# huggingface/distil-whisper

Hardware: AMD Instinct MI355X
Metric: training audio-seconds/s (distil-large-v3 student, 30 s clips) (higher is better)
Workload: dtype bf16

## Files before the change

### distil_whisper_amd/build.py

```python
import os
import subprocess
import sys

HERE = os.path.dirname(os.path.abspath(__file__))
CSRC = os.path.join(HERE, "csrc")
LIB = os.path.join(HERE, "libdwamd.so")
SOURCES = ["gemm.hip", "gemm_tile256.hip", "gemm_tile128.hip", "gemm_wp8_nn.hip", "gemm_wp8_nt.hip", "gemm_wp8_m320.hip", "gemm_wp8_m128.hip",
           "gemm_wp16_nn.hip", "gemm_wp16_tt.hip", "gemm_wp16_small.hip", "gemm_skinny.hip", "attention.hip", "norm.hip", "loss.hip", "logmel.hip", "elementwise.hip", "optim.hip", "decode.hip", "align.hip", "score.hip", "dropout.hip"]
FLAGS = ["--offload-arch=gfx950", "-O3", "-std=c++17", "-fPIC", "-ffp-contract=fast", "-munsafe-fp-atomics"]


def kernels_sha16() -> str:
    import hashlib
    h = hashlib.sha256()
    files = sorted(os.path.join(CSRC, f) for f in os.listdir(CSRC) if f.endswith((".hip", ".h")))
    files.append(os.path.join(HERE, "..", "include", "dwamd.h"))
    for f in files:
        h.update(os.path.basename(f).encode())
        with open(f, "rb") as fh:
            h.update(fh.read())
    return h.hexdigest()[:16]


def _stale(obj, deps):
    if not os.path.exists(obj):
        return True
    t = os.path.getmtime(obj)
    return any(os.path.getmtime(d) > t for d in deps)


# ... 33 lines not shown
```

### distil_whisper_amd/csrc/gemm.hip

```cpp
#include "gemm_common.h"
#include <mutex>
#include <unordered_map>

bool dw_gemm_skinny_ok(const GemmP& p, int trans_a, int trans_b);
int dw_gemm_skinny_launch(const GemmP& p, hipStream_t s);
int dw_gemm_tile256_launch(const GemmP& p, int ta, int tb, hipStream_t s);
int dw_gemm_tile128_launch(const GemmP& p, int ta, int tb, hipStream_t s);
int dw_gemm_wp8_nn_launch(const GemmP& p, hipStream_t s);
int dw_gemm_wp8_nt_launch(const GemmP& p, hipStream_t s);
int dw_gemm_wp8_nn320_launch(const GemmP& p, hipStream_t s);
int dw_gemm_wp8_nt320_launch(const GemmP& p, hipStream_t s);
int dw_gemm_wp8_nn128_launch(const GemmP& p, hipStream_t s);
int dw_gemm_wp8_nt128_launch(const GemmP& p, hipStream_t s);
int dw_gemm_wp16_nn_launch(const GemmP& p, hipStream_t s);
int dw_gemm_wp16_tt_launch(const GemmP& p, hipStream_t s);
int dw_gemm_wp16_nn_small_launch(const GemmP& p, hipStream_t s);
int dw_gemm_wp16_nt_small_launch(const GemmP& p, hipStream_t s);

extern int g_attn_bwd_stage;
extern int g_attn_decode;
extern int g_attn_ablate;
extern int g_attn_fwd_waves;
extern int g_attn_fwd_pipe;
extern int g_attn_plain_order;
extern int g_attn_defer;
extern int g_attn_bwd_waves;
extern int g_logmel_mfma;
extern int g_decode_fuse_off;
extern int g_skinny_wide;
extern int g_ln_variant;
enum { GEMM_RULE = 0,
       GEMM_REFERENCE = 1,
       GEMM_FORCE_320 = 2 };
static int g_gemm_mode = GEMM_RULE;
int g_gemm_strip = 0;
int g_gemm_cus = 256;
static int g_gemm_stage_next = 1;
static int g_gemm_dynamic = 1;
static int g_gemm_small_m = 1;
static int g_gemm_row_tail = 1;

static int* gemm_sched_slot(hipStream_t s) {
    static std::mutex mu;
    static std::unordered_map<hipStream_t, int*> slots;
    std::lock_guard<std::mutex> lock(mu);
    auto it = slots.find(s);
    if (it != slots.end()) return it->second;
    hipStreamCaptureStatus st = hipStreamCaptureStatusNone;
    if (hipStreamIsCapturing(s, &st) != hipSuccess || st != hipStreamCaptureStatusNone) { (void)hipGetLastError(); return nullptr; }
    int* ptr = nullptr;
    if (hipMalloc((void**)&ptr, 64) != hipSuccess || hipMemsetAsync(ptr, 0, 64, s) != hipSuccess) { (void)hipGetLastError(); return nullptr; }
    slots[s] = ptr;
    return ptr;
}
int g_gemm_strip_budget = 4;
extern "C" int dw_debug_set(int key, int value) {
    if (key == 0) { if (value < GEMM_RULE || value > GEMM_FORCE_320) return DW_EINVAL; g_gemm_mode = value; return DW_OK; }
    if (key == 1) { g_gemm_strip = value; return DW_OK; }
    if (key == 3) { g_attn_bwd_stage = value; return DW_OK; }
    if (key == 4) { g_attn_decode = value; return DW_OK; }
    if (key == 5) { g_logmel_mfma = value; return DW_OK; }
    if (key == 6) { g_gemm_strip_budget = value; return DW_OK; }
    if (key == 7) { g_decode_fuse_off = value; return DW_OK; }
    if (key == 8) { g_skinny_wide = value; return DW_OK; }
    if (key == 10) { g_gemm_dynamic = value; return DW_OK; }
    if (key == 11) { g_gemm_stage_next = value; return DW_OK; }
    if (key == 17) { g_attn_bwd_waves = value; return DW_OK; }
    if (key == 21) { g_ln_variant = value; return DW_OK; }
    if (key == 22) { g_gemm_row_tail = value; return DW_OK; }
    if (key == 25) { if (value < 0 || value > 1) return DW_EINVAL; g_gemm_small_m = value; return DW_OK; }
    if (key == 26) { g_attn_fwd_pipe = value; return DW_OK; }
    if (key == 18) { g_attn_plain_order = value; return DW_OK; }
    if (key == 23) { if (value < 0 || value > 64) return DW_EINVAL; g_attn_defer = value; return DW_OK; }
    if (key == 16) { g_attn_fwd_waves = value; return DW_OK; }
    if (key == 15) { g_attn_ablate = value; return DW_OK; }
    if (key == 9) { if (value < 8 || value > 256 || (value & 7)) return DW_EINVAL; g_gemm_cus = value; return DW_OK; }
    return DW_EINVAL;
}

__global__ __launch_bounds__(256) void reduce_slices_kernel(const float* part, long stride, int slices, float* out,
                                                            long n, int accumulate) {
    const long i = ((long)blockIdx.x * 256 + threadIdx.x) * 4;
    if (i >= n) return;
    f32x4 acc = accumulate ? *(const f32x4*)(out + i) : f32x4{0.f, 0.f, 0.f, 0.f};
    for (int s = 0; s < slices; ++s) {
        const f32x4 v = *(const f32x4*)(part + s * stride + i);
#pragma unroll
        for (int e = 0; e < 4; ++e) acc[e] += v[e];
    }
    *(f32x4*)(out + i) = acc;
}

// ... 28 lines not shown
                                   int rows, int cols, int accumulate, void* stream) {
    DW_CLEAR_ERR();
    if (!part || !out || slices < 1 || rows <= 0 || cols <= 0 || (cols & 3) || (ld_part & 3) || (ld_out & 3) || (slice_stride & 3) ||
        ld_part < cols || ld_out < cols || ((uintptr_t)part & 15) || ((uintptr_t)out & 15))
        return DW_EINVAL;
    const long n = (long)rows * (cols / 4);
    hipLaunchKernelGGL(reduce_slices_ld_kernel, dim3((n + 255) / 256), dim3(256), 0, (hipStream_t)stream, part, (long)slice_stride,
                       (long)ld_part, slices, out, (long)ld_out, rows, cols / 4, accumulate);
    DW_CHECK_LAUNCH();
    return DW_OK;
}

enum GemmKernel {
    K_SKINNY,
    K_TILE128,
    K_TILE256,
    K_WP8_M128,
    K_WP16_SMALL,
    K_WP8_320,
    K_WP16_NN,
    K_WP8_NN,
    K_WP8_NT,
    K_WP16_TT,
};

static GemmKernel gemm_choose(const DwGemm* g, const GemmP& p) {
    const bool ta = g->trans_a, tb = g->trans_b, nn = !ta && !tb;
    const bool one_slice = p.split_k == 1 && !p.atomic;
    const bool ref = g_gemm_mode == GEMM_REFERENCE;
    const bool res_f32 = g->r && g->r_dtype == DW_F32 && g->c_dtype == DW_F32;
    const long cus = g_gemm_cus, tn = (g->n + 255) / 256;
    const long t256 = (long)((g->m + 255) / 256) * tn;
    const bool fits320 = !ta && one_slice && g->m % 320 == 0 && g->n % 256 == 0;
    int tile = g->tile;
    if ((tile == 0 || tile == 16) && dw_gemm_skinny_ok(p, ta, tb)) return K_SKINNY;
    bool one_round_320 = false, small_m_256 = false;
    if (tile != 128 && tile != 256) {
        tile = t256 >= 512 ? 256 : 128;
        if (tile == 128 && !ref && g_gemm_small_m && !ta && one_slice) {
            const long r128 = (((long)(g->m + 127) / 128) * tn + cus - 1) / cus;
            const long r256 = (t256 + cus - 1) / cus;
            const long r320 = fits320 ? ((long)(g->m / 320) * tn + cus - 1) / cus : 0;
            const long c128 = r128 * 100, c256 = r256 * 165, c320 = fits320 ? r320 * 205 : (1L << 40);
            if (c320 <= c128 && c320 <= c256) { tile = 256; one_round_320 = true; }
            else if (c256 <= c128) { tile = 256; small_m_256 = true; }
            else return K_WP8_M128;
        }
    }
    if (tile == 256 && g->tile != 256 && nn && res_f32 && g->k <= 1024 && one_slice) tile = 128;
    if (tile == 128) return K_TILE128;
    const long spanA = ta ? (long)g->k * g->lda * 2 : 256L * g->lda * 2 + (long)g->k * 2;
    const long spanB = tb ? (long)g->k * g->ldb * 2 : 256L * g->ldb * 2 + (long)g->k * 2;
    if (ref || spanA >= 0x7fffffffL || spanB >= 0x7fffffffL) return K_TILE256;
    if (small_m_256) return K_WP16_SMALL;
    if (fits320 && (one_round_320 || g_gemm_mode == GEMM_FORCE_320)) return K_WP8_320;
    if (nn && g->k <= 2560 && g->n >= 3840 && !g->r && !g->z_out && !g->zgrad_in && g->c_dtype != DW_F32) return K_WP16_NN;
    if (fits320) {
        const long r256 = (((g->m + 255) / 256) * tn + cus - 1) / cus * 4;
        const long r320 = ((g->m / 320) * tn + cus - 1) / cus * 5;
        if (tb ? r320 < r256 && !g->zgrad_in : r320 <= r256) return K_WP8_320;
    }
    if (nn) return res_f32 && g->k <= 2560 ? K_TILE256 : K_WP8_NN;
    if (!ta) return K_WP8_NT;
    if (tb) return K_WP16_TT;
    return K_TILE256;
}

extern "C" int dw_gemm_bf16(const DwGemm* g, void* stream) {
    DW_CLEAR_ERR();
    if (!g || (!g->a && !g->ln_x) || !g->b || !g->c) return DW_EINVAL;
    if (g->m <= 0 || g->n <= 0 || g->k <= 0 || (g->k & 63)) return DW_EINVAL;
    if ((g->lda & 7) || (g->ldb & 7)) return DW_EINVAL;
    if ((g->a && ((uintptr_t)g->a & 15)) || ((uintptr_t)g->b & 15)) return DW_EINVAL;
    if (g->trans_a && g->lda < ((g->m + 7) & ~7)) return DW_EINVAL;
    if (g->trans_b && g->ldb < ((g->n + 7) & ~7)) return DW_EINVAL;
    GemmP p;
    p.a = (const bf16*)g->a; p.b = (const bf16*)g->b; p.c = g->c; p.bias = g->bias;
    p.z_out = (bf16*)g->z_out; p.zgrad = (const bf16*)g->zgrad_in; p.r = g->r;
    p.lda = g->lda; p.ldb = g->ldb; p.ldc = g->ldc; p.ldz = g->ldz; p.ldzg = g->ldzg; p.ldr = g->ldr;
    p.m = g->m; p.n = g->n; p.k = g->k;
    p.act = g->act; p.c_dtype = g->c_dtype; p.r_dtype = g->r_dtype; p.r_row_mod = g->r_row_mod;
    p.round_res = g->round_res; p.tiles_n = 0; p.nwg = 0;
    p.split_k = g->split_k > 1 ? g->split_k : 1;
    p.atomic = g->atomic_acc ? 1 : 0;
    if (p.split_k > (g->k >> 6)) p.split_k = g->k >> 6;
    p.slice_stride = 0;
    p.sched = nullptr;
// ... 29 lines not shown
        if (g->r) v = v && ((uintptr_t)g->r % (g->r_dtype == DW_F32 ? 16 : 8)) == 0 && (g->ldr & 3) == 0;
        p.vec = v ? 1 : 0;
    }
    hipStream_t s = (hipStream_t)stream;
    if (g->tile == 16 && !dw_gemm_skinny_ok(p, g->trans_a, g->trans_b)) return DW_EINVAL;
    const GemmKernel kern = gemm_choose(g, p);
    if (kern == K_SKINNY) {
        if (g->colsum_out) return DW_EINVAL;
        return dw_gemm_skinny_launch(p, s);
    }
    if (fused) return DW_EINVAL;
    if (g->tile == 129 && (g->trans_a || p.split_k != 1 || p.atomic)) return DW_EINVAL;
    if (kern == K_TILE128) return dw_gemm_tile128_launch(p, g->trans_a, g->trans_b, s);
    p.strip = g_gemm_strip;
    if (g_gemm_dynamic) p.sched = gemm_sched_slot(s);
    if (kern == K_WP8_M128) return g->trans_b ? dw_gemm_wp8_nt128_launch(p, s) : dw_gemm_wp8_nn128_launch(p, s);
    if (g->k <= 1024) p.stage_next |= 128;
    switch (kern) {
    case K_WP16_SMALL: return g->trans_b ? dw_gemm_wp16_nt_small_launch(p, s) : dw_gemm_wp16_nn_small_launch(p, s);
    case K_WP8_320: return g->trans_b ? dw_gemm_wp8_nt320_launch(p, s) : dw_gemm_wp8_nn320_launch(p, s);
    case K_WP8_NN: return dw_gemm_wp8_nn_launch(p, s);
    case K_WP8_NT: return dw_gemm_wp8_nt_launch(p, s);
    case K_WP16_TT: return dw_gemm_wp16_tt_launch(p, s);
    case K_WP16_NN: {
        const int tm_full = p.m / 256, rem = p.m - tm_full * 256;
        const long tn = (p.n + 255) / 256;
        const long rounds_all = ((long)(tm_full + 1) * tn + g_gemm_cus - 1) / g_gemm_cus;
        const long rounds_full = ((long)tm_full * tn + g_gemm_cus - 1) / g_gemm_cus;
        if (g_gemm_row_tail && g->tile != 256 && rem > 0 && rem <= 128 && tm_full > 0 && rounds_full < rounds_all && !p.colsum) {
            GemmP q1 = p, q2 = p;
            q1.m = tm_full * 256;
            const size_t es = p.c_dtype == DW_F32 ? 4 : 2;
            q2.m = rem;
            q2.a = p.a + (long)q1.m * p.lda;
            q2.c = (char*)p.c + (size_t)q1.m * p.ldc * es;
            q2.sched = nullptr;
            const int rc1 = dw_gemm_wp16_nn_launch(q1, s);
            if (rc1 != DW_OK) return rc1;
            return dw_gemm_tile128_launch(q2, 0, 0, s);
        }
        return dw_gemm_wp16_nn_launch(p, s);
    }
    default: return dw_gemm_tile256_launch(p, g->trans_a, g->trans_b, s);
    }
}
```

### distil_whisper_amd/csrc/gemm_common.h

```cpp
#pragma once
#include "common.h"
#include "../../include/dwamd.h"

struct GemmP {
    const bf16* a;
    const bf16* b;
    void* c;
    const float* bias;
    bf16* z_out;
    const bf16* zgrad;
    const void* r;
    long lda, ldb, ldc, ldz, ldzg, ldr;
    int m, n, k;
    int act, c_dtype, r_dtype, r_row_mod, round_res;
    int tiles_n, nwg;
    int strip;
    int split_k, atomic;
    int vec;
    long slice_stride;
    const void* ln_x;
    const float* ln_g;
    const float* ln_b;
    long ld_lnx;
    int ln_x_dtype;
// ... 87 lines not shown
    int strip = id / per_strip;
    int within = id - strip * per_strip;
    int width = sw;
    const int full = p.tiles_n - (nstrips - 1) * sw;
    if (strip >= nstrips - 1) {
        strip = nstrips - 1;
        within = id - strip * per_strip;
        width = full;
    }
    tm = within / width;
    tn = strip * sw + (within - tm * width);
}

extern int g_gemm_strip_budget;
extern int g_gemm_cus;
inline int gemm_strip_width(int k, int tiles_n, int override_) {
    if (override_ > 0) return override_;
    const long tile_bytes = 256L * k * 2;
    int sw = (int)(((long)g_gemm_strip_budget << 19) / tile_bytes);
    if (sw < 2 || sw >= tiles_n) sw = tiles_n;
    return sw;
}

template <int BX>
__device__ __forceinline__ bf16x8 frag_kmajor(const char* tile, int x, int kk, int lane) {
    constexpr int RB = BX * 2;
    const int g = lane >> 4, p = lane & 15;
    const int col = x + ((g & 1) << 4) + ((p & 3) << 2);
    const int k0 = kk * 16 + ((g >> 1) << 3) + (p >> 2);
    const int ls = col >> 3;
    const int inb = (p & 1) << 3;
    const int sw = ((p >> 2) & 3) << 2;
    const char* a0 = tile + k0 * RB + ((ls ^ sw) << 4) + inb;
    const char* a1 = a0 + 4 * RB;
    bf16x4 lo = __builtin_amdgcn_ds_read_tr16_b64_v4bf16((lds_bf16x4_t*)a0);
    bf16x4 hi = __builtin_amdgcn_ds_read_tr16_b64_v4bf16((lds_bf16x4_t*)a1);
    bf16x8 r;
    r[0] = lo[0]; r[1] = lo[1]; r[2] = lo[2]; r[3] = lo[3];
    r[4] = hi[0]; r[5] = hi[1]; r[6] = hi[2]; r[7] = hi[3];
    return r;
}


typedef __attribute__((ext_vector_type(4))) unsigned u32x4;
enum { EPI_BIAS = 1, EPI_ZBF16 = 2, EPI_GELU = 4, EPI_STOREG = 8, EPI_ZG16 = 16, EPI_ZGBF = 32, EPI_RES = 64, EPI_RES_F32 = 128,
       EPI_ROUND = 256, EPI_OUT_F32 = 512, EPI_COLSUM = 1024 };
__device__ __forceinline__ int gemm_epi_flavour(const GemmP& p) {
    return (p.bias ? EPI_BIAS : 0) | ((p.z_out && !p.zg_f16) ? EPI_ZBF16 : 0) | (p.act == 1 ? EPI_GELU : 0) |
           ((p.z_out && p.zg_f16) ? EPI_STOREG : 0) | ((p.zgrad && p.zg_f16) ? EPI_ZG16 : 0) |
           ((p.zgrad && !p.zg_f16) ? EPI_ZGBF : 0) | (p.r ? EPI_RES : 0) | ((p.r && p.r_dtype == DW_F32) ? EPI_RES_F32 : 0) |
           ((p.r && p.round_res) ? EPI_ROUND : 0) | (p.c_dtype == DW_F32 ? EPI_OUT_F32 : 0) | (p.colsum ? EPI_COLSUM : 0);
}
template <class T>
__device__ __forceinline__ void gemm_store_out(T* dst, const T& v) {
    __builtin_nontemporal_store(v, dst);
// ... 82 lines not shown
    }
}

template <int LPR>
__device__ __forceinline__ void gemm_colsum_flush(const GemmP& p, float (&cs)[4], int lane, int n) {
#pragma unroll
    for (int e = 0; e < 4; ++e) {
#pragma unroll
        for (int o = LPR; o < 64; o <<= 1) cs[e] += __shfl_xor(cs[e], o);
    }
    if (lane < LPR) {
#pragma unroll
        for (int e = 0; e < 4; ++e)
            if (n + e < p.n) atomicAdd(p.colsum + n + e, cs[e]);
    }
}

struct GemmNoHook { __device__ __forceinline__ void operator()() const {} };
__device__ __forceinline__ void gemm_lds_barrier() {
    asm volatile("s_waitcnt lgkmcnt(0)" ::: "memory");
    __builtin_amdgcn_s_barrier();
    asm volatile("" ::: "memory");
}
template <int FM, int FN, int TN, int PFDIST = 0, class Hook = GemmNoHook, bool SWZ = false, int LAY = 32, int JOFF = 0, class Acc = f32x16[FM][FN]>
__device__ __forceinline__ void gemm_epilogue(const GemmP& p, Acc& acc, char* smem, int wave, int lane,
                                              int m0_, int wm0_, int n0_, int wn0_, int ks_, Hook hook = Hook(),
                                              const float* lds_bias = nullptr) {
    static_assert(!SWZ || TN == 64, "swizzled patch: 16 slots of 16 bytes per row");
    asm volatile("" : "+v"(lane));
    const int m0 = __builtin_amdgcn_readfirstlane(m0_), wm0 = __builtin_amdgcn_readfirstlane(wm0_);
    const int n0 = __builtin_amdgcn_readfirstlane(n0_), wn0 = __builtin_amdgcn_readfirstlane(wn0_);
    const int ks = __builtin_amdgcn_readfirstlane(ks_);
    constexpr int PLD = SWZ ? TN : TN + 4;
    constexpr int LPR = TN / 4;
    constexpr int RPI = 64 / LPR;
    constexpr int NIT = 32 / RPI;
    float* patch = (float*)smem + wave * (32 * PLD);
    const int hi = lane >> 5, ln = lane & 31;
    const int lrow = LAY == 32 ? ln : (lane & 15);
    const int lcol = LAY == 32 ? hi * 4 : (lane >> 4) * 4;
    auto qrow = [](int q) constexpr -> int { return LAY == 32 ? 0 : (q / (FN * 2)) * 16; };
    auto qcol = [](int q) constexpr -> int { return LAY == 32 ? (q / 4) * 32 + (q % 4) * 8 : (q % (FN * 2)) * 16; };
    auto quad = [&](auto ic, auto qc) __attribute__((always_inline)) -> f32x4 {
        constexpr int i = decltype(ic)::value, q = decltype(qc)::value;
        f32x4 v4;
        if constexpr (LAY == 32) {
            constexpr int j = q / 4, g = q % 4;
// ... 178 lines not shown
                    const bf16x2 r0 = __builtin_convertvector(p[0], bf16x2), r1 = __builtin_convertvector(p[1], bf16x2);
                    u32x2 o;
                    o[0] = __builtin_bit_cast(unsigned, r0); o[1] = __builtin_bit_cast(unsigned, r1);
                    *(u32x2*)(wr + qrow(q) * PRS + qcol(q) * 2) = o;
                });
                });
                flush(c_u, p.ldc, l_c16, ic);
                if constexpr (HAS_G) {
                    static_for<0, FN * 4>([&](auto qc) __attribute__((always_inline)) {
                        constexpr int q = decltype(qc)::value;
                        *(f16x4*)(wr + qrow(q) * PRS + qcol(q) * 2) = gq[q];
                    });
                    flush(z_u, p.ldz, l_z16, ic);
                }
            });
        };
        const bool ok16 = SWZ && p.c_dtype != DW_F32 && ((uintptr_t)p.c & 15) == 0 && (p.ldc & 7) == 0 && (!p.bias || lds_bias) &&
                          (!p.z_out || (((uintptr_t)p.z_out & 15) == 0 && (p.ldz & 7) == 0));
#define DW_EPI_CASE16(F)                                                                             \
    case (F):                                                                                        \
        if constexpr (SWZ) { if (ok16) { walk16(std::integral_constant<int, (F)>{}); return; } }      \
        walk(std::integral_constant<int, (F)>{}); return
#define DW_EPI_CASE(F) case (F): walk(std::integral_constant<int, (F)>{}); return
        if constexpr (FM == 4 || FM == 2) {
            switch (gemm_epi_flavour(p)) {
                DW_EPI_CASE16(0);
                DW_EPI_CASE16(EPI_BIAS);
                DW_EPI_CASE16(EPI_BIAS | EPI_GELU);
                DW_EPI_CASE(EPI_BIAS | EPI_GELU | EPI_STOREG);
                DW_EPI_CASE(EPI_BIAS | EPI_RES | EPI_RES_F32 | EPI_ROUND | EPI_OUT_F32);
                DW_EPI_CASE(EPI_BIAS | EPI_RES | EPI_ROUND);
                DW_EPI_CASE(EPI_ZG16);
                DW_EPI_CASE(EPI_ZG16 | EPI_COLSUM);
                DW_EPI_CASE(EPI_RES | EPI_RES_F32 | EPI_ROUND | EPI_OUT_F32);
                DW_EPI_CASE(EPI_OUT_F32);
                default: break;
            }
        } else {
            if constexpr (FM == 5) {
                switch (gemm_epi_flavour(p)) {
                    DW_EPI_CASE16(0);
                    DW_EPI_CASE16(EPI_BIAS);
                    DW_EPI_CASE16(EPI_BIAS | EPI_GELU);
                    DW_EPI_CASE(EPI_BIAS | EPI_GELU | EPI_STOREG);
                    DW_EPI_CASE(EPI_BIAS | EPI_RES | EPI_RES_F32 | EPI_ROUND | EPI_OUT_F32);
                    DW_EPI_CASE(EPI_BIAS | EPI_RES | EPI_ROUND);
                    default: break;
// ... 78 lines not shown
```

### distil_whisper_amd/csrc/gemm_wp.h

```cpp
#pragma once
#include "gemm_common.h"

#define PINF(f) asm volatile("" : "+v"((f)[0]), "+v"((f)[1]), "+v"((f)[2]), "+v"((f)[3]))
#define PINF2(f) asm volatile("" : "+v"((f)[0]), "+v"((f)[1]))
#define PIN_SET(set)                                                                                              \
    do {          \
        if constexpr (FM == 4 && FN == 2)                                                                                 \
            asm volatile("" : "+v"(af[set][0]), "+v"(af[set][1]), "+v"(af[set][2]), "+v"(af[set][3]), "+v"(bfr[set][0]), "+v"(bfr[set][1]));   \
        else if constexpr (FM == 5 && FN == 2)                                                                            \
            asm volatile("" : "+v"(af[set][0]), "+v"(af[set][1]), "+v"(af[set][2]), "+v"(af[set][3]), "+v"(af[set][4]), "+v"(bfr[set][0]),     \
                         "+v"(bfr[set][1]));                                                                              \
        else {                                                                                                            \
            if constexpr (FM == 4) PINF(af[set]);                                                                         \
            else if constexpr (FM == 5) { PINF(af[set]); asm volatile("" : "+v"(af[set][4])); }                          \
            else PINF2(af[set]);                                                                                          \
            if constexpr (FN == 4) PINF(bfr[set]); else PINF2(bfr[set]);                                                  \
        }                                                                                                                 \
    } while (0)

typedef __attribute__((ext_vector_type(4))) int i32x4_t;
__device__ __forceinline__ i32x4_t wp_rsrc(const void* base) {
    const unsigned long long a = (unsigned long long)base;
    i32x4_t r;
    r[0] = (int)(unsigned)a; r[1] = (int)((unsigned)(a >> 32) & 0xffffu); r[2] = 0x7fffffff; r[3] = 0x00020000;
// ... 9 lines not shown
}
__device__ __forceinline__ void wp_dma16u(const i32x4_t& rsrc, unsigned lds_addr, unsigned voffset, int soffset) {
    asm volatile("s_mov_b32 m0, %0\n\ts_nop 0\n\tbuffer_load_dwordx4 %1, %2, %3 offen lds"
                 :: "s"(lds_addr), "v"(voffset), "s"(rsrc), "s"(soffset));
}
template <int IMM>
__device__ __forceinline__ void wp_dma16p(const i32x4_t& rsrc, unsigned lds_base, unsigned voffset, int kbase, int piece_off) {
    int so;
    asm volatile("s_add_u32 m0, %1, %5\n\ts_add_u32 %0, %4, %6\n\tbuffer_load_dwordx4 %2, %3, %0 offen lds"
                 : "=&s"(so) : "s"(lds_base), "v"(voffset), "s"(rsrc), "s"(kbase), "i"(IMM), "s"(piece_off) : "scc");
}
template <int IMM>
__device__ __forceinline__ void wp_dma16i(const i32x4_t& rsrc, unsigned lds_base, unsigned voffset, int soffset) {
    asm volatile("s_add_u32 m0, %0, %4\n\ts_nop 0\n\tbuffer_load_dwordx4 %1, %2, %3 offen lds"
                 :: "s"(lds_base), "v"(voffset), "s"(rsrc), "s"(soffset), "i"(IMM) : "scc");
}

template <bool TA, bool TB, int WM, int WN, bool ASMDMA, int DBG, int BM, int NST>
__global__ __launch_bounds__(64 * WM * WN, WM * WN / 4) void gemm_wp_kernel(const GemmP p) {
    static_assert(ASMDMA && DBG == 0, "one build of the loop: inline-assembly operand DMA, no ablation");
    constexpr int BN = 256, NW = WM * WN, FM = BM / WM / 32, FN = BN / WN / 32, TN = BN / WN;
    static_assert(NST == 2 || (NST == 3 && BM < 256), "three stages: the 128-row tile");
    static_assert(NW * 32 * (TN + 4) * 4 <= 2 * (BM + BN) * 128, "epilogue patches must fit the operand buffers");
    static_assert(BM == 256 || !TA, "the k-major A image is built for 256-row tiles");
    constexpr int CPA = BM / 8 / NW, CPB = BN / 8 / NW;
    constexpr int CP = CPB;
    constexpr bool UNI = BM == 320;
    constexpr int EPF = 4;
    static_assert(CPA * 8 * NW == BM && CPB * 8 * NW == BN && CPA <= 8 && CPB <= 8, "piece split");
    constexpr int NA0 = (CPA + 1) / 2, NB0 = CPB / 2;
    constexpr int NH0 = NA0 + NB0, NH1 = CPA + CPB - NH0;
    constexpr int STAGE = (BM + BN) * 128;
    __shared__ __attribute__((aligned(1024))) char smem[NST * STAGE];
    __shared__ __attribute__((aligned(1024))) float bias_lds[BN];

    const int tid = threadIdx.x;
    const int lane = tid & 63;
    const int wave = __builtin_amdgcn_readfirstlane(tid >> 6);
    const int wm0 = (wave / WN) * (BM / WM), wn0 = (wave % WN) * TN;
    const unsigned smem_w = wp_lds_addr(smem) + (unsigned)(wave * 1024);

    __shared__ int job_slot[2];
    GemmJobs jobs;
    gemm_jobs_begin(p, jobs, job_slot);
    bool prefetched = false;
    while (jobs.cur < jobs.cnt) {
        int lane_k = lane;
        asm volatile("" : "+v"(lane_k));
        gemm_jobs_prefetch(p, jobs, job_slot);
        int tm, tn, ks;
        gemm_job_decode(p, jobs.start + jobs.cur, tm, tn, ks);
        const int m0 = tm * BM, n0 = tn * BN;

        unsigned offA[8], offB[8];
        const bf16* gA;
        const bf16* gB;
        int stepA, stepB;
        if (!TA) {
            gA = p.a + (long)m0 * p.lda;
            stepA = 128;
#pragma unroll
            for (int i = 0; i < CPA; ++i) {
                const int row = (wave + i * NW) * 8 + (lane_k >> 3);
                const int ls = (lane_k & 7) ^ swz7(row);
                const int grow = m0 + row < p.m ? row : p.m - 1 - m0;
                offA[i] = (unsigned)((grow * p.lda + ls * 8) * 2);
            }
        } else {
            gA = p.a + m0;
            stepA = 128 * (int)p.lda;
#pragma unroll
            for (int i = 0; i < CPA; ++i) {
                const int krow = (wave + i * NW) * 2 + (lane_k >> 5);
                const int ls = (lane_k & 31) ^ ((krow & 3) << 2);
                const int gcol = m0 + ls * 8 < p.m ? ls * 8 : 0;
                offA[i] = (unsigned)((krow * p.lda + gcol) * 2);
            }
        }
        if (!TB) {
            gB = p.b + (long)n0 * p.ldb;
            stepB = 128;
#pragma unroll
            for (int i = 0; i < CP; ++i) {
                const int row = (wave + i * NW) * 8 + (lane_k >> 3);
                const int ls = (lane_k & 7) ^ swz7(row);
                const int grow = n0 + row < p.n ? row : p.n - 1 - n0;
                offB[i] = (unsigned)((grow * p.ldb + ls * 8) * 2);
            }
        } else {
            gB = p.b + n0;
            stepB = 128 * (int)p.ldb;
#pragma unroll
            for (int i = 0; i < CP; ++i) {
                const int krow = (wave + i * NW) * 2 + (lane_k >> 5);
                const int ls = (lane_k & 31) ^ ((krow & 3) << 2);
                const int gcol = n0 + ls * 8 < p.n ? ls * 8 : 0;
                offB[i] = (unsigned)((krow * p.ldb + gcol) * 2);
            }
        }
        const int pieceA = UNI ? NW * (TA ? 2 : 8) * (int)p.lda * 2 : 0;
        const int pieceB = UNI ? NW * (TB ? 2 : 8) * (int)p.ldb * 2 : 0;
        int nt = p.k >> 6;
        {
            const int base = nt / p.split_k, rem = nt - base * p.split_k;
            const int first = ks * base + (ks < rem ? ks : rem);
            nt = base + (ks < rem ? 1 : 0);
            gA = (const bf16*)((const char*)gA + (long)first * stepA);
            gB = (const bf16*)((const char*)gB + (long)first * stepB);
        }
        const i32x4_t rsA = wp_rsrc(gA), rsB = wp_rsrc(gB);
        int kA = 0, kB = 0;

        f32x16 acc[FM][FN];
#pragma unroll
        for (int i = 0; i < FM; ++i)
#pragma unroll
            for (int j = 0; j < FN; ++j)
#pragma unroll
                for (int r = 0; r < 16; ++r) acc[i][j][r] = 0.f;

        auto dma1x = [&](const i32x4_t& ra, const i32x4_t& rb, auto hc, auto jc, int buf) __attribute__((always_inline)) {
            constexpr int h = decltype(hc)::value, j = decltype(jc)::value;
            constexpr int na = h ? CPA - NA0 : NA0, nb = h ? CPB - NB0 : NB0, nmin = na < nb ? na : nb;
            constexpr bool isA = j < 2 * nmin ? (j & 1) == 0 : na > nb;
            constexpr int idx = j < 2 * nmin ? j / 2 : j - nmin;
            constexpr int i = (isA ? (h ? NA0 : 0) : (h ? NB0 : 0)) + idx;
            static_assert(j < na + nb, "load index");
            const unsigned lb = smem_w + (unsigned)(buf * STAGE);
            if constexpr (UNI) {
                if constexpr (isA) wp_dma16p<i * (NW * 1024)>(ra, lb, offA[0], kA, i * pieceA);
                else wp_dma16p<i * (NW * 1024) + BM * 128>(rb, lb, offB[0], kB, i * pieceB);
            } else {
                if constexpr (isA) wp_dma16i<i * (NW * 1024)>(ra, lb, offA[i], kA);
                else wp_dma16i<i * (NW * 1024) + BM * 128>(rb, lb, offB[i], kB);
            }
        };
        auto dma1 = [&](auto hc, auto jc, int buf) __attribute__((always_inline)) { dma1x(rsA, rsB, hc, jc, buf); };
        auto dma = [&](auto hc, int buf) __attribute__((always_inline)) {
            static_for<0, (decltype(hc)::value ? NH1 : NH0)>([&](auto jc) __attribute__((always_inline)) { dma1(hc, jc, buf); });
        };
        bf16x8 af[2][FM], bfr[2][FN];
        auto frags = [&](auto sc, auto kc, int buf) {
            constexpr int set = decltype(sc)::value, kk = decltype(kc)::value;
            const char* tA = smem + buf * STAGE;
            const char* tB = tA + BM * 128;
#pragma unroll
            for (int i = 0; i < FM; ++i) {
                if (TA) af[set][i] = frag_kmajor<BM>(tA, wm0 + i * 32, kk, lane_k);
                else af[set][i] = frag_rows(tA, (wm0 >> 5) + i, kk, lane_k);
            }
#pragma unroll
            for (int j = 0; j < FN; ++j) {
                if (TB) bfr[set][j] = frag_kmajor<BN>(tB, wn0 + j * 32, kk, lane_k);
                else bfr[set][j] = frag_rows(tB, (wn0 >> 5) + j, kk, lane_k);
            }
        };
// ... 120 lines not shown
        if (nt >= 2) { body(std::true_type{}, std::false_type{}, t); ++t; }
        body(std::false_type{}, std::false_type{}, t);
        }

        prefetched = false;
        if constexpr (TN == 64 && BM >= 256) {
            const int nxt = jobs.dynamic ? job_slot[(jobs.iter + 1) & 1] : jobs.cur + jobs.step;
            if ((p.stage_next & 128) && (nt & 1) == 0 && nt >= 2 && nxt < jobs.cnt && tile_in && !p.zgrad && !p.r) {
                int tm2, tn2, ks2;
                gemm_job_decode(p, jobs.start + nxt, tm2, tn2, ks2);
                if ((tm2 + 1) * BM <= p.m && (tn2 + 1) * BN <= p.n) {
                    const int ntall = p.k >> 6, base2 = ntall / p.split_k, rem2 = ntall - base2 * p.split_k;
                    const long first2 = (long)ks2 * base2 + (ks2 < rem2 ? ks2 : rem2);
                    const char* a2 = (const char*)(TA ? p.a + tm2 * BM : p.a + (long)tm2 * BM * p.lda) + first2 * stepA;
                    const char* b2 = (const char*)(TB ? p.b + tn2 * BN : p.b + (long)tn2 * BN * p.ldb) + first2 * stepB;
                    const i32x4_t ra2 = wp_rsrc(a2), rb2 = wp_rsrc(b2);
                    kA = 0; kB = 0;
                    static_for<0, NH0>([&](auto jc) __attribute__((always_inline)) { dma1x(ra2, rb2, I0{}, jc, 0); });
                    static_for<0, NH1>([&](auto jc) __attribute__((always_inline)) { dma1x(ra2, rb2, I1{}, jc, 0); });
                    prefetched = true;
                }
            }
        }
        gemm_epilogue<FM, FN, TN, (BM == 320 ? EPF : 8), GemmNoHook, TN == 64>(p, acc, smem + (TN == 64 && STAGE >= NW * 8192 ? STAGE : 0), wave, lane, m0,
                                                                          wm0, n0, wn0, ks, GemmNoHook(), tile_in ? bias_lds : nullptr);
        gemm_lds_barrier();
        gemm_jobs_advance(jobs, job_slot);
    }
    gemm_jobs_end(p, jobs);
}

template <bool TA, bool TB, int WM, int WN, int BM = 256, int NST = 2>
static int launch_wp(const GemmP& p0, hipStream_t s) {
    GemmP p = p0;
    const int tiles_m = (p.m + BM - 1) / BM;
    p.tiles_n = (p.n + 255) / 256;
    p.nwg = tiles_m * p.tiles_n;
    p.strip = gemm_strip_width(p.k, p.tiles_n, p.strip);
    int nblk = p.nwg * p.split_k;
    if (nblk > g_gemm_cus) nblk = g_gemm_cus;
    hipLaunchKernelGGL((gemm_wp_kernel<TA, TB, WM, WN, true, 0, BM, NST>), dim3(nblk), dim3(64 * WM * WN), 0, s, p);
    DW_CHECK_LAUNCH();
    return DW_OK;
}
```

### distil_whisper_amd/ops_hip.py

```python
import ctypes as C
import math
import os

import torch

_HERE = os.path.dirname(os.path.abspath(__file__))
LIB_PATH = os.path.join(_HERE, "libdwamd.so")

DW_F32, DW_BF16 = 0, 1


class DwGemm(C.Structure):
    _fields_ = [
        ("a", C.c_void_p), ("b", C.c_void_p), ("c", C.c_void_p), ("bias", C.c_void_p), ("z_out", C.c_void_p),
        ("zgrad_in", C.c_void_p), ("r", C.c_void_p),
        ("lda", C.c_int64), ("ldb", C.c_int64), ("ldc", C.c_int64), ("ldz", C.c_int64), ("ldzg", C.c_int64),
        ("ldr", C.c_int64),
        ("m", C.c_int32), ("n", C.c_int32), ("k", C.c_int32),
        ("trans_a", C.c_int32), ("trans_b", C.c_int32), ("act", C.c_int32), ("c_dtype", C.c_int32),
        ("r_dtype", C.c_int32), ("r_row_mod", C.c_int32), ("round_res", C.c_int32), ("tile", C.c_int32),
        ("split_k", C.c_int32), ("atomic_acc", C.c_int32), ("slice_stride", C.c_int64),
        ("ln_x", C.c_void_p), ("ln_gamma", C.c_void_p), ("ln_beta", C.c_void_p), ("kv_out", C.c_void_p),
        ("ld_lnx", C.c_int64), ("kv_ld", C.c_int64),
        ("ln_x_dtype", C.c_int32), ("kv_split", C.c_int32), ("kv_rows_per_batch", C.c_int32),
# ... 5 lines not shown
class DwDecoderLayer(C.Structure):
    _fields_ = [(n, C.c_void_p) for n in (
        "ln1_g", "ln1_b", "wqkv", "bqkv", "wo", "bo", "ln2_g", "ln2_b", "wq", "bq", "wo2", "bo2", "ln3_g", "ln3_b",
        "w1", "b1", "w2", "b2", "self_kv", "cross_kv")]


class DwDecodeStep(C.Structure):
    _fields_ = [(n, C.c_int32) for n in (
        "batch", "n_new", "d_model", "heads", "ffn", "n_layers", "src_len", "max_len", "t", "vocab", "ldv",
        "stream_dtype", "cross_kv_ld")] + [(n, C.c_void_p) for n in (
            "ids", "tok_emb", "pos_emb", "lnf_g", "lnf_b", "lm_head", "layers", "x", "h", "qkv", "o", "a", "logits")]


_SIGS = {
    "dw_version": ([], C.c_int),
    "dw_decode_step": ([C.POINTER(DwDecodeStep), C.c_void_p], C.c_int),
    "dw_logmel": ([C.c_void_p, C.c_int, C.c_int, C.c_void_p, C.c_int, C.c_void_p, C.c_void_p, C.c_void_p, C.c_void_p,
                   C.c_void_p], C.c_int),
    "dw_gemm_bf16": ([C.POINTER(DwGemm), C.c_void_p], C.c_int),
    "dw_layernorm_fwd": ([C.c_void_p, C.c_int, C.c_void_p, C.c_void_p, C.c_void_p, C.c_void_p, C.c_void_p, C.c_int,
                          C.c_int, C.c_float, C.c_void_p], C.c_int),
    "dw_layernorm_bwd": ([C.c_void_p, C.c_void_p, C.c_int, C.c_void_p, C.c_void_p, C.c_void_p, C.c_void_p, C.c_int,
                          C.c_void_p, C.c_void_p, C.c_void_p, C.c_void_p, C.c_int, C.c_int, C.c_void_p], C.c_int),
    "dw_reduce_slices_ld": ([C.c_void_p, C.c_int64, C.c_int64, C.c_int, C.c_void_p, C.c_int64, C.c_int, C.c_int, C.c_int, C.c_void_p], C.c_int),
    "dw_layernorm_fwd_ld": ([C.c_void_p, C.c_int, C.c_void_p, C.c_void_p, C.c_void_p, C.c_void_p, C.c_void_p, C.c_int,
                             C.c_int, C.c_float, C.c_int64, C.c_int64, C.c_void_p], C.c_int),
    "dw_layernorm_bwd_ld": ([C.c_void_p, C.c_void_p, C.c_int, C.c_void_p, C.c_void_p, C.c_void_p, C.c_void_p, C.c_int,
                             C.c_void_p, C.c_void_p, C.c_void_p, C.c_void_p, C.c_int, C.c_int] + [C.c_int64] * 4 + [C.c_void_p], C.c_int),
    "dw_attn_fwd": ([C.c_void_p] * 5 + [C.c_int] * 4 + [C.c_int64] * 4 + [C.c_int, C.c_float, C.c_void_p], C.c_int),
    "dw_attn_fwd_ex": ([C.c_void_p] * 5 + [C.c_int] * 4 + [C.c_int64] * 6 + [C.c_int, C.c_float, C.c_void_p], C.c_int),
    "dw_attn_fwd_varlen": ([C.c_void_p] * 4 + [C.c_int] * 4 + [C.c_int64] * 4 + [C.c_void_p] * 4 + [C.c_int, C.c_int64, C.c_int, C.c_float,
                                                                                                           C.c_void_p], C.c_int),
    "dw_attn_bwd": ([C.c_void_p] * 10 + [C.c_int] * 4 + [C.c_int64] * 8 + [C.c_int, C.c_float, C.c_void_p], C.c_int),
    "dw_attn_bwd_ex": ([C.c_void_p] * 10 + [C.c_int] * 4 + [C.c_int64] * 8 + [C.c_int, C.c_float] + [C.c_void_p] * 3, C.c_int),
    "dw_distill_loss": ([C.c_void_p, C.c_void_p, C.c_void_p, C.c_int, C.c_int, C.c_int64, C.c_float, C.c_float,
                         C.c_float, C.c_float, C.c_void_p, C.c_void_p, C.c_void_p, C.c_void_p, C.c_void_p,
                         C.c_void_p], C.c_int),
    "dw_distill_loss_w": ([C.c_void_p, C.c_void_p, C.c_void_p, C.c_int, C.c_int, C.c_int64, C.c_float, C.c_void_p,
                           C.c_float, C.c_void_p, C.c_void_p, C.c_void_p, C.c_void_p, C.c_void_p, C.c_void_p], C.c_int),
    "dw_embed_fwd": ([C.c_void_p, C.c_void_p, C.c_void_p, C.c_int, C.c_void_p, C.c_int, C.c_int, C.c_int, C.c_int,
                      C.c_void_p], C.c_int),
    "dw_embed_bwd": ([C.c_void_p, C.c_void_p, C.c_void_p, C.c_void_p, C.c_int, C.c_int, C.c_int, C.c_void_p], C.c_int),
    "dw_im2col_mel": ([C.c_void_p, C.c_void_p, C.c_int, C.c_int, C.c_int, C.c_int, C.c_void_p], C.c_int),
    "dw_im2col_s2": ([C.c_void_p, C.c_void_p, C.c_int, C.c_int, C.c_int, C.c_void_p], C.c_int),
    "dw_col2im_s2_gelu_bwd": ([C.c_void_p, C.c_void_p, C.c_void_p, C.c_int, C.c_int, C.c_int, C.c_void_p], C.c_int),
    "dw_gelu_bwd": ([C.c_void_p, C.c_int, C.c_void_p, C.c_void_p, C.c_int64, C.c_void_p], C.c_int),
# ... 49 lines not shown
    for name, (args, res) in _SIGS.items():
        fn = getattr(lib, name)
        fn.argtypes = args
        fn.restype = res
    return lib


def _dt(t):
    if t.dtype == torch.float32:
        return DW_F32
    if t.dtype == torch.bfloat16:
        return DW_BF16
    raise TypeError(f"unsupported dtype {t.dtype}")


def _p(t):
    return None if t is None else t.data_ptr()


def dropout_threshold(p):
    return min(2**32 - 1, int(round(float(p) * 2.0**32)))


def _rup4(x):
    return (int(x) + 3) // 4 * 4


class HipOps:

    name = "hip"
    lowp = torch.bfloat16

    def __init__(self, device="cuda:0"):
        if not torch.cuda.is_available():
            raise RuntimeError("HipOps needs a ROCm GPU (torch.cuda.is_available() is False); there is no CPU path.")
        self.lib = load_library()
        self.device = torch.device(device)
        i = torch.arange(400, dtype=torch.float64)
        ang = 2.0 * math.pi * i / 400.0
        self._twiddle = torch.stack([torch.cos(ang), torch.sin(ang)], 1).to(torch.float32).contiguous().to(self.device)
        self._window = torch.hann_window(400, periodic=True, dtype=torch.float64).to(torch.float32).to(self.device)
        self.profile = None
        self._prof_events = []
        self.profile_detail = False

    def _stream(self):
# ... 72 lines not shown
            Kb, N = b.shape
        else:
            N, Kb = b.shape
        assert K == Kb, (a.shape, b.shape, trans_a, trans_b)
        if out is None:
            out = self.empty((M, N + out_row_pad), self.lowp if out_dtype is None else out_dtype)
            if out_row_pad:
                out = out[:, :N]
        assert out.shape == (M, N) and out.stride(1) == 1
        g = DwGemm()
        g.a, g.b, g.c = a.data_ptr(), b.data_ptr(), out.data_ptr()
        g.lda, g.ldb, g.ldc = a.stride(0), b.stride(0), out.stride(0)
        g.m, g.n, g.k = M, N, K
        g.trans_a, g.trans_b = int(trans_a), int(trans_b)
        g.act = int(act)
        g.c_dtype = _dt(out)
        g.tile = int(tile) if tile else 0
        tile_key = g.tile if tile or M <= 64 else self.pick_tile(M, N)
        ws = None
        if atomic_acc:
            assert out.dtype == torch.float32 and bias is None and residual is None and not want_z and zgrad is None
            if not tile:
                g.tile = tile_key = 256
            tiles = ((M + g.tile - 1) // g.tile) * ((N + g.tile - 1) // g.tile)
            nt = K // 64
            if split_k:
                sk = int(split_k)
            else:
                best, sk = -1.0, 1
                for cand in range(1, max(1, min(16, nt // 16)) + 1):
                    jobs = tiles * cand
                    eff = jobs / (-(-jobs // 256) * 256) - 0.004 * cand
                    if eff > best + 1e-9:
                        best, sk = eff, cand
            sk = max(1, min(sk, nt // 16))
            if sk > 1 and out.stride(1) == 1 and N % 4 == 0 and out.stride(0) % 4 == 0:
                ldw = N + self.wgrad_slab_pad
                ws = self.empty((sk, M, ldw), torch.float32)
                g.c, g.ldc = ws.data_ptr(), ldw
                g.split_k, g.slice_stride = sk, M * ldw
            elif overwrite:
                g.atomic_acc, g.split_k = 0, 1
            else:
                g.atomic_acc, g.split_k = 1, 1
        if ln is not None:
            gamma, beta = ln[0], ln[1]
            assert a.dtype in (torch.float32, torch.bfloat16) and not trans_a
            assert gamma.dtype == torch.float32 and beta.dtype == torch.float32 and gamma.numel() == K == beta.numel()
            g.a, g.ln_x, g.ld_lnx, g.ln_x_dtype = None, a.data_ptr(), a.stride(0), _dt(a)
            g.ln_gamma, g.ln_beta, g.ln_eps = gamma.data_ptr(), beta.data_ptr(), float(ln[2]) if len(ln) > 2 else 1e-5
        if kv_append is not None:
            cache, split, rpb, pitch, row0 = kv_append
            assert cache.dtype == torch.bfloat16 and cache.stride(-1) == 1
            g.kv_out, g.kv_ld, g.kv_split = cache.data_ptr(), N - split, int(split)
            g.kv_rows_per_batch, g.kv_batch_pitch, g.kv_row0 = int(rpb), int(pitch), int(row0)
        z = None
        if bias is not None:
            assert bias.dtype == torch.float32 and bias.numel() == N and bias.is_contiguous()
# ... 454 lines not shown
```

### include/dwamd.h

```cpp
#ifndef DWAMD_H
#define DWAMD_H
#include <stdint.h>
#ifdef __cplusplus
extern "C" {
#endif

#define DW_OK 0
#define DW_EINVAL (-1)
#define DW_EUNSUP (-2)

#define DW_F32 0
#define DW_BF16 1

int dw_version(void);

int dw_logmel(const float* audio, int batch, int n_samples, const float* mel_filters, int n_mels,
              const float* twiddle, const float* window, float* out, float* clipmax, void* stream);

typedef struct DwGemm {
    const void* a;
    const void* b;
    void* c;
    const float* bias;
    void* z_out;
// ... 6 lines not shown
    int32_t c_dtype;
    int32_t r_dtype;
    int32_t r_row_mod;
    int32_t round_res;
    int32_t tile;
    int32_t split_k;
    int32_t atomic_acc;
    int64_t slice_stride;
    const void* ln_x;
    const float* ln_gamma;
    const float* ln_beta;
    void* kv_out;
    int64_t ld_lnx, kv_ld;
    int32_t ln_x_dtype;
    int32_t kv_split, kv_rows_per_batch, kv_batch_pitch, kv_row0;
    float ln_eps;
    int32_t z_is_gelu_grad;
    float* colsum_out;
} DwGemm;
int dw_gemm_bf16(const DwGemm* g, void* stream);
int dw_reduce_slices(const float* part, int64_t stride, int slices, float* out, int64_t n, int accumulate, void* stream);
int dw_reduce_slices_ld(const float* part, int64_t slice_stride, int64_t ld_part, int slices, float* out, int64_t ld_out,
                        int rows, int cols, int accumulate, void* stream);

int dw_layernorm_fwd(const void* x, int x_dtype, const float* gamma, const float* beta, void* y, float* mean,
                     float* rstd, int rows, int cols, float eps, void* stream);
int dw_layernorm_bwd(const void* dy_bf16, const void* x, int x_dtype, const float* mean, const float* rstd,
                     const float* gamma, float* dres, int accumulate, float* dgamma, float* dbeta, void* dres_lowp,
                     float* dres_colsum, int rows, int cols, void* stream);
int dw_layernorm_fwd_ld(const void* x, int x_dtype, const float* gamma, const float* beta, void* y, float* mean,
                        float* rstd, int rows, int cols, float eps, int64_t ldx, int64_t ldy, void* stream);
int dw_layernorm_bwd_ld(const void* dy_bf16, const void* x, int x_dtype, const float* mean, const float* rstd,
                        const float* gamma, float* dres, int accumulate, float* dgamma, float* dbeta, void* dres_lowp,
                        float* dres_colsum, int rows, int cols, int64_t lddy, int64_t ldx, int64_t lddres,
                        int64_t ldlowp, void* stream);

int dw_attn_fwd(const void* q, const void* k, const void* v, void* o, float* lse, int B, int H, int Lq, int Lk,
                int64_t ldq, int64_t ldk, int64_t ldv, int64_t ldo, int causal, float scale, void* stream);
int dw_attn_fwd_ex(const void* q, const void* k, const void* v, void* o, float* lse, int B, int H, int Lq, int Lk,
                   int64_t ldq, int64_t ldk, int64_t ldv, int64_t ldo, int64_t q_batch_rows, int64_t kv_batch_rows,
                   int causal, float scale, void* stream);
int dw_attn_fwd_varlen(const void* q, const void* k, const void* v, void* o, int n_seq, int H, int max_q, int Lk, int64_t ldq,
                       int64_t ldk, int64_t ldv, int64_t ldo, const int32_t* q_start, const int32_t* q_len,
                       const int32_t* kv_start, const int32_t* kv_len, int kv_batches, int64_t kv_batch_rows, int causal,
                       float scale, void* stream);
int dw_attn_bwd(const void* q, const void* k, const void* v, const void* o, const void* d_o, const float* lse,
// ... 117 lines not shown
```

Baseline: 2875.

## Add 320-row transposed-A/B weight-gradient GEMM kernel with split-k planning

```diff
diff --git a/distil_whisper_amd/build.py b/distil_whisper_amd/build.py
--- a/distil_whisper_amd/build.py
+++ b/distil_whisper_amd/build.py
@@ -5,7 +5,7 @@
 HERE = os.path.dirname(os.path.abspath(__file__))
 CSRC = os.path.join(HERE, "csrc")
 LIB = os.path.join(HERE, "libdwamd.so")
-SOURCES = ["gemm.hip", "gemm_tile256.hip", "gemm_tile128.hip", "gemm_wp8_nn.hip", "gemm_wp8_nt.hip", "gemm_wp8_m320.hip", "gemm_wp8_m128.hip",
+SOURCES = ["gemm.hip", "gemm_tile256.hip", "gemm_tile128.hip", "gemm_wp8_nn.hip", "gemm_wp8_nt.hip", "gemm_wp8_m320.hip", "gemm_wp8_tt320.hip", "gemm_wp8_m128.hip",
            "gemm_wp16_nn.hip", "gemm_wp16_tt.hip", "gemm_wp16_small.hip", "gemm_skinny.hip", "attention.hip", "norm.hip", "loss.hip", "logmel.hip", "elementwise.hip", "optim.hip", "decode.hip", "align.hip", "score.hip", "dropout.hip"]
 FLAGS = ["--offload-arch=gfx950", "-O3", "-std=c++17", "-fPIC", "-ffp-contract=fast", "-munsafe-fp-atomics"]
 
diff --git a/distil_whisper_amd/csrc/gemm.hip b/distil_whisper_amd/csrc/gemm.hip
--- a/distil_whisper_amd/csrc/gemm.hip
+++ b/distil_whisper_amd/csrc/gemm.hip
@@ -10,6 +10,7 @@
 int dw_gemm_wp8_nt_launch(const GemmP& p, hipStream_t s);
 int dw_gemm_wp8_nn320_launch(const GemmP& p, hipStream_t s);
 int dw_gemm_wp8_nt320_launch(const GemmP& p, hipStream_t s);
+int dw_gemm_wp8_tt320_launch(const GemmP& p, hipStream_t s);
 int dw_gemm_wp8_nn128_launch(const GemmP& p, hipStream_t s);
 int dw_gemm_wp8_nt128_launch(const GemmP& p, hipStream_t s);
 int dw_gemm_wp16_nn_launch(const GemmP& p, hipStream_t s);
@@ -38,6 +39,7 @@
 static int g_gemm_stage_next = 1;
 static int g_gemm_dynamic = 1;
 static int g_gemm_small_m = 1;
+static int g_gemm_wgrad320 = -1;
 static int g_gemm_row_tail = 1;
 
 static int* gemm_sched_slot(hipStream_t s) {
@@ -68,6 +70,7 @@
     if (key == 17) { g_attn_bwd_waves = value; return DW_OK; }
     if (key == 21) { g_ln_variant = value; return DW_OK; }
     if (key == 22) { g_gemm_row_tail = value; return DW_OK; }
+    if (key == 27) { if (value < -1 || value > 1) return DW_EINVAL; g_gemm_wgrad320 = value; return DW_OK; }
     if (key == 25) { if (value < 0 || value > 1) return DW_EINVAL; g_gemm_small_m = value; return DW_OK; }
     if (key == 26) { g_attn_fwd_pipe = value; return DW_OK; }
     if (key == 18) { g_attn_plain_order = value; return DW_OK; }
@@ -142,7 +145,19 @@
     K_WP8_NN,
     K_WP8_NT,
     K_WP16_TT,
+    K_WP8_TT320,
 };
+
+static int gemm_wgrad_rows(long m, long n, long k, long lda, long ldb) {
+    if (g_gemm_mode == GEMM_REFERENCE || g_gemm_wgrad320 == 0) return 256;
+    if (m <= 0 || n <= 0 || m % 320 != 0 || n % 256 != 0) return 256;
+    if (k * lda * 2 >= 0x7fffffffL || k * ldb * 2 >= 0x7fffffffL) return 256;
+    if (g_gemm_wgrad320 == 1) return 320;
+    return (m / 320) * (n / 256) >= 60 ? 320 : 256;
+}
+extern "C" int dw_gemm_wgrad_rows(int64_t m, int64_t n, int64_t k, int64_t lda, int64_t ldb) {
+    return gemm_wgrad_rows((long)m, (long)n, (long)k, (long)lda, (long)ldb);
+}
 
 static GemmKernel gemm_choose(const DwGemm* g, const GemmP& p) {
     const bool ta = g->trans_a, tb = g->trans_b, nn = !ta && !tb;
@@ -182,7 +197,11 @@
     }
     if (nn) return res_f32 && g->k <= 2560 ? K_TILE256 : K_WP8_NN;
     if (!ta) return K_WP8_NT;
-    if (tb) return K_WP16_TT;
+    if (tb) {
+        const bool bare_f32 = g->c_dtype == DW_F32 && !g->bias && !g->z_out && !g->zgrad_in && !g->r && !g->act && !g->colsum_out;
+        if (bare_f32 && gemm_wgrad_rows(g->m, g->n, g->k, g->lda, g->ldb) == 320) return K_WP8_TT320;
+        return K_WP16_TT;
+    }
     return K_TILE256;
 }
 
@@ -258,6 +277,7 @@
     case K_WP8_NN: return dw_gemm_wp8_nn_launch(p, s);
     case K_WP8_NT: return dw_gemm_wp8_nt_launch(p, s);
     case K_WP16_TT: return dw_gemm_wp16_tt_launch(p, s);
+    case K_WP8_TT320: return dw_gemm_wp8_tt320_launch(p, s);
     case K_WP16_NN: {
         const int tm_full = p.m / 256, rem = p.m - tm_full * 256;
         const long tn = (p.n + 255) / 256;
diff --git a/distil_whisper_amd/csrc/gemm_common.h b/distil_whisper_amd/csrc/gemm_common.h
--- a/distil_whisper_amd/csrc/gemm_common.h
+++ b/distil_whisper_amd/csrc/gemm_common.h
@@ -133,6 +133,7 @@
     return sw;
 }
 
+__device__ __forceinline__ int swk_w(int krow) { return ((krow >> 1) & 1) << 2; }
 template <int BX>
 __device__ __forceinline__ bf16x8 frag_kmajor(const char* tile, int x, int kk, int lane) {
     constexpr int RB = BX * 2;
@@ -141,7 +142,7 @@
     const int k0 = kk * 16 + ((g >> 1) << 3) + (p >> 2);
     const int ls = col >> 3;
     const int inb = (p & 1) << 3;
-    const int sw = ((p >> 2) & 3) << 2;
+    const int sw = BX == 320 ? ((p >> 3) & 1) << 2 : ((p >> 2) & 3) << 2;
     const char* a0 = tile + k0 * RB + ((ls ^ sw) << 4) + inb;
     const char* a1 = a0 + 4 * RB;
     bf16x4 lo = __builtin_amdgcn_ds_read_tr16_b64_v4bf16((lds_bf16x4_t*)a0);
@@ -270,7 +271,8 @@
     __builtin_amdgcn_s_barrier();
     asm volatile("" ::: "memory");
 }
-template <int FM, int FN, int TN, int PFDIST = 0, class Hook = GemmNoHook, bool SWZ = false, int LAY = 32, int JOFF = 0, class Acc = f32x16[FM][FN]>
+template <int FM, int FN, int TN, int PFDIST = 0, class Hook = GemmNoHook, bool SWZ = false, int LAY = 32, int JOFF = 0, int ONLY = -1,
+          class Acc = f32x16[FM][FN]>
 __device__ __forceinline__ void gemm_epilogue(const GemmP& p, Acc& acc, char* smem, int wave, int lane,
                                               int m0_, int wm0_, int n0_, int wn0_, int ks_, Hook hook = Hook(),
                                               const float* lds_bias = nullptr) {
@@ -495,7 +497,10 @@
         if constexpr (SWZ) { if (ok16) { walk16(std::integral_constant<int, (F)>{}); return; } }      \
         walk(std::integral_constant<int, (F)>{}); return
 #define DW_EPI_CASE(F) case (F): walk(std::integral_constant<int, (F)>{}); return
-        if constexpr (FM == 4 || FM == 2) {
+        if constexpr (ONLY >= 0) {
+            walk(std::integral_constant<int, ONLY>{});
+            return;
+        } else if constexpr (FM == 4 || FM == 2) {
             switch (gemm_epi_flavour(p)) {
                 DW_EPI_CASE16(0);
                 DW_EPI_CASE16(EPI_BIAS);
diff --git a/distil_whisper_amd/csrc/gemm_wp.h b/distil_whisper_amd/csrc/gemm_wp.h
--- a/distil_whisper_amd/csrc/gemm_wp.h
+++ b/distil_whisper_amd/csrc/gemm_wp.h
@@ -55,10 +55,11 @@
     constexpr int BN = 256, NW = WM * WN, FM = BM / WM / 32, FN = BN / WN / 32, TN = BN / WN;
     static_assert(NST == 2 || (NST == 3 && BM < 256), "three stages: the 128-row tile");
     static_assert(NW * 32 * (TN + 4) * 4 <= 2 * (BM + BN) * 128, "epilogue patches must fit the operand buffers");
-    static_assert(BM == 256 || !TA, "the k-major A image is built for 256-row tiles");
+    static_assert(!TA || BM == 256 || BM == 320, "the k-major A image is built for 256- and 320-row tiles");
     constexpr int CPA = BM / 8 / NW, CPB = BN / 8 / NW;
     constexpr int CP = CPB;
     constexpr bool UNI = BM == 320;
+    constexpr bool UNIA = UNI && !TA;
     constexpr int EPF = 4;
     static_assert(CPA * 8 * NW == BM && CPB * 8 * NW == BN && CPA <= 8 && CPB <= 8, "piece split");
     constexpr int NA0 = (CPA + 1) / 2, NB0 = CPB / 2;
@@ -99,6 +100,16 @@
                 const int grow = m0 + row < p.m ? row : p.m - 1 - m0;
                 offA[i] = (unsigned)((grow * p.lda + ls * 8) * 2);
             }
+        } else if (BM == 320) {
+            gA = p.a + m0;
+            stepA = 128 * (int)p.lda;
+#pragma unroll
+            for (int i = 0; i < CPA; ++i) {
+                const int L = (wave + i * NW) * 64 + lane_k;
+                const int krow = L / 40;
+                const int ls = (L - krow * 40) ^ swk_w(krow);
+                offA[i] = (unsigned)((krow * p.lda + ls * 8) * 2);
+            }
         } else {
             gA = p.a + m0;
             stepA = 128 * (int)p.lda;
@@ -131,7 +142,7 @@
                 offB[i] = (unsigned)((krow * p.ldb + gcol) * 2);
             }
         }
-        const int pieceA = UNI ? NW * (TA ? 2 : 8) * (int)p.lda * 2 : 0;
+        const int pieceA = UNIA ? NW * 8 * (int)p.lda * 2 : 0;
         const int pieceB = UNI ? NW * (TB ? 2 : 8) * (int)p.ldb * 2 : 0;
         int nt = p.k >> 6;
         {
@@ -160,11 +171,11 @@
             constexpr int i = (isA ? (h ? NA0 : 0) : (h ? NB0 : 0)) + idx;
             static_assert(j < na + nb, "load index");
             const unsigned lb = smem_w + (unsigned)(buf * STAGE);
-            if constexpr (UNI) {
-                if constexpr (isA) wp_dma16p<i * (NW * 1024)>(ra, lb, offA[0], kA, i * pieceA);
-                else wp_dma16p<i * (NW * 1024) + BM * 128>(rb, lb, offB[0], kB, i * pieceB);
+            if constexpr (isA) {
+                if constexpr (UNIA) wp_dma16p<i * (NW * 1024)>(ra, lb, offA[0], kA, i * pieceA);
+                else wp_dma16i<i * (NW * 1024)>(ra, lb, offA[i], kA);
             } else {
-                if constexpr (isA) wp_dma16i<i * (NW * 1024)>(ra, lb, offA[i], kA);
+                if constexpr (UNI) wp_dma16p<i * (NW * 1024) + BM * 128>(rb, lb, offB[0], kB, i * pieceB);
                 else wp_dma16i<i * (NW * 1024) + BM * 128>(rb, lb, offB[i], kB);
             }
         };
@@ -331,7 +342,8 @@
                 }
             }
         }
-        gemm_epilogue<FM, FN, TN, (BM == 320 ? EPF : 8), GemmNoHook, TN == 64>(p, acc, smem + (TN == 64 && STAGE >= NW * 8192 ? STAGE : 0), wave, lane, m0,
+        constexpr int ONLY = TA && TB && BM == 320 ? EPI_OUT_F32 : -1;
+        gemm_epilogue<FM, FN, TN, (BM == 320 ? EPF : 8), GemmNoHook, TN == 64, 32, 0, ONLY>(p, acc, smem + (TN == 64 && STAGE >= NW * 8192 ? STAGE : 0), wave, lane, m0,
                                                                           wm0, n0, wn0, ks, GemmNoHook(), tile_in ? bias_lds : nullptr);
         gemm_lds_barrier();
         gemm_jobs_advance(jobs, job_slot);
diff --git a/distil_whisper_amd/csrc/gemm_wp8_tt320.hip b/distil_whisper_amd/csrc/gemm_wp8_tt320.hip
--- /dev/null
+++ b/distil_whisper_amd/csrc/gemm_wp8_tt320.hip
@@ -0,0 +1,2 @@
+#include "gemm_wp.h"
+int dw_gemm_wp8_tt320_launch(const GemmP& p, hipStream_t s) { return launch_wp<true, true, 2, 4, 320>(p, s); }
diff --git a/distil_whisper_amd/ops_hip.py b/distil_whisper_amd/ops_hip.py
--- a/distil_whisper_amd/ops_hip.py
+++ b/distil_whisper_amd/ops_hip.py
@@ -51,6 +51,7 @@
                           C.c_int, C.c_float, C.c_void_p], C.c_int),
     "dw_layernorm_bwd": ([C.c_void_p, C.c_void_p, C.c_int, C.c_void_p, C.c_void_p, C.c_void_p, C.c_void_p, C.c_int,
                           C.c_void_p, C.c_void_p, C.c_void_p, C.c_void_p, C.c_int, C.c_int, C.c_void_p], C.c_int),
+    "dw_gemm_wgrad_rows": ([C.c_int64] * 5, C.c_int),
     "dw_reduce_slices_ld": ([C.c_void_p, C.c_int64, C.c_int64, C.c_int, C.c_void_p, C.c_int64, C.c_int, C.c_int, C.c_int, C.c_void_p], C.c_int),
     "dw_layernorm_fwd_ld": ([C.c_void_p, C.c_int, C.c_void_p, C.c_void_p, C.c_void_p, C.c_void_p, C.c_void_p, C.c_int,
                              C.c_int, C.c_float, C.c_int64, C.c_int64, C.c_void_p], C.c_int),
@@ -146,6 +147,25 @@
     return min(2**32 - 1, int(round(float(p) * 2.0**32)))
 
 
+WGRAD_SLICE_PENALTY = {256: 0.004, 320: 0.018}
+
+
+def wgrad_slice_plan(M, N, K, rows, tile=256, split_k=0, cus=256):
+    tiles = ((M + rows - 1) // rows) * ((N + tile - 1) // tile)
+    nt = K // 64
+    if split_k:
+        sk = int(split_k)
+    else:
+        pen = WGRAD_SLICE_PENALTY.get(rows, WGRAD_SLICE_PENALTY[256])
+        best, sk = -1.0, 1
+        for cand in range(1, max(1, min(16, nt // 16)) + 1):
+            jobs = tiles * cand
+            eff = jobs / (-(-jobs // cus) * cus) - pen * cand
+            if eff > best + 1e-9:
+                best, sk = eff, cand
+    return tiles, max(1, min(sk, nt // 16))
+
+
 def _rup4(x):
     return (int(x) + 3) // 4 * 4
 
@@ -264,18 +284,10 @@
             assert out.dtype == torch.float32 and bias is None and residual is None and not want_z and zgrad is None
             if not tile:
                 g.tile = tile_key = 256
-            tiles = ((M + g.tile - 1) // g.tile) * ((N + g.tile - 1) // g.tile)
-            nt = K // 64
-            if split_k:
-                sk = int(split_k)
-            else:
-                best, sk = -1.0, 1
-                for cand in range(1, max(1, min(16, nt // 16)) + 1):
-                    jobs = tiles * cand
-                    eff = jobs / (-(-jobs // 256) * 256) - 0.004 * cand
-                    if eff > best + 1e-9:
-                        best, sk = eff, cand
-            sk = max(1, min(sk, nt // 16))
+            rows = g.tile
+            if g.tile == 256 and trans_a and trans_b:
+                rows = self.lib.dw_gemm_wgrad_rows(M, N, K, a.stride(0), b.stride(0))
+            _, sk = wgrad_slice_plan(M, N, K, rows, g.tile, split_k=split_k)
             if sk > 1 and out.stride(1) == 1 and N % 4 == 0 and out.stride(0) % 4 == 0:
                 ldw = N + self.wgrad_slab_pad
                 ws = self.empty((sk, M, ldw), torch.float32)
diff --git a/include/dwamd.h b/include/dwamd.h
--- a/include/dwamd.h
+++ b/include/dwamd.h
@@ -52,6 +52,7 @@
 int dw_reduce_slices(const float* part, int64_t stride, int slices, float* out, int64_t n, int accumulate, void* stream);
 int dw_reduce_slices_ld(const float* part, int64_t slice_stride, int64_t ld_part, int slices, float* out, int64_t ld_out,
                         int rows, int cols, int accumulate, void* stream);
+int dw_gemm_wgrad_rows(int64_t m, int64_t n, int64_t k, int64_t lda, int64_t ldb);
 
 int dw_layernorm_fwd(const void* x, int x_dtype, const float* gamma, const float* beta, void* y, float* mean,
                      float* rstd, int rows, int cols, float eps, void* stream);
```

After: 2894 (median of 6 runs). Within noise of the previous version (+0.7%).
